# onesamblack/distributed-torch-horovod-gcp

Hardware: NVIDIA H100
Metric: images/sec (whole job, device-timed, max over ranks) ResNet-50 synthetic ImageNet training (higher is better)
Workload: dtype bf16

## Files before the change

### distributed_torch_horovod_gcp_b200/csrc/conv_sm90.cu

```cuda
#include <cuda.h>
#include <cuda_bf16.h>
#include <cuda_runtime.h>
#include <limits.h>
#include <stdint.h>
#include <stdio.h>
#include <stdlib.h>
#include <string.h>

#include "sm90_common.cuh"

namespace {

constexpr int MAX_TAPS = 9;
constexpr int MAX_CLASSES = 4;

struct ConvTap {
  int amap;
  int dw, dh;
  int wcol;
};
struct ConvClass {
  int ntaps;
  int out_map;
  ConvTap taps[MAX_TAPS];
};
struct ConvParams {
  GemmParams g;
  int num_classes;
  int kc_per_tap;
  int bw, bh, bn;
  int sw, sh;
  int tiles_w, tiles_h, tiles_n;
  int num_taps_total;
  int out_w, out_h, out_n;
  ConvClass cls[MAX_CLASSES];
};
struct alignas(64) ConvMaps {
  CUtensorMap a[4];
  CUtensorMap b;
  CUtensorMap out[4];
};

enum { MODE_FPROP = 0, MODE_DGRAD = 1, MODE_WGRAD = 2 };

template <int BN, int MODE>
struct ConvWork {
  static constexpr bool kStats = MODE == MODE_FPROP, kSplitK = MODE == MODE_WGRAD;
  static constexpr bool B_MN = MODE != MODE_FPROP;
  const ConvMaps& maps;
  const ConvParams& p;
  int nnb, pix_tiles, tiles, items, kb_per_split;

  __device__ ConvWork(const ConvMaps& maps_, const ConvParams& p_)
      : maps(maps_), p(p_), nnb(p_.g.num_n_blocks), pix_tiles(p_.tiles_w * p_.tiles_h * p_.tiles_n),
        tiles(MODE == MODE_WGRAD ? p_.g.num_m_blocks * nnb * p_.num_taps_total : p_.num_classes * pix_tiles * nnb),
        items(tiles * p_.g.splits),
        kb_per_split(MODE == MODE_WGRAD ? (pix_tiles + p_.g.splits - 1) / p_.g.splits : 0) {}
  __device__ void prefetch() const {
    for (int i = 0; i < 4; ++i) tma_prefetch_desc(&maps.a[i]);
    tma_prefetch_desc(&maps.b);
    for (int i = 0; i < 4; ++i) tma_prefetch_desc(&maps.out[i]);
  }
  __device__ int num_kb(int w) const {
    if (MODE != MODE_WGRAD) return p.cls[(w / nnb) / pix_tiles].ntaps * p.kc_per_tap;
    const int kb0 = (w / tiles) * kb_per_split;
    return min(kb0 + kb_per_split, pix_tiles) - kb0;
  }
  template <class Next>
  __device__ void load(int w, Next& next) const {
    if (MODE != MODE_WGRAD) {
      const int nt = w % nnb;
      const int rest = w / nnb;
      const int mt = rest % pix_tiles;
      const ConvClass& cl = p.cls[rest / pix_tiles];
      const int w0 = (mt % p.tiles_w) * p.bw;
      const int h0 = ((mt / p.tiles_w) % p.tiles_h) * p.bh;
      const int n0 = (mt / (p.tiles_w * p.tiles_h)) * p.bn;
      const int n_idx = nt * BN;
      for (int t = 0; t < cl.ntaps; ++t) {
        const ConvTap tap = cl.taps[t];
        for (int kc = 0; kc < p.kc_per_tap; ++kc) {
          const Stage s = next();
          tma_load_4d(&maps.a[tap.amap], s.bar, s.a, kc * BLOCK_K, w0 + tap.dw, h0 + tap.dh, n0);
          if (!B_MN) {
            tma_load_2d(&maps.b, s.bar, s.b, tap.wcol + kc * BLOCK_K, n_idx);
          } else {
#pragma unroll
            for (int c = 0; c < BN / 64; ++c)
              tma_load_2d(&maps.b, s.bar, s.b + c * (BLOCK_K * 128), tap.wcol + n_idx + 64 * c, kc * BLOCK_K);
          }
        }
      }
    } else {
      const int tile = w % tiles, split = w / tiles;
      const ConvTap tap = p.cls[0].taps[tile % p.num_taps_total];
      const int mn = tile / p.num_taps_total;
      const int m_idx = (mn / nnb) * BLOCK_M;
      const int n_idx = (mn % nnb) * BN;
      const int kb0 = split * kb_per_split;
      const int kb1 = min(kb0 + kb_per_split, pix_tiles);
      for (int kb = kb0; kb < kb1; ++kb) {
        const int w0 = (kb % p.tiles_w) * p.bw;
        const int h0 = ((kb / p.tiles_w) % p.tiles_h) * p.bh;
        const int n0 = (kb / (p.tiles_w * p.tiles_h)) * p.bn;
        const Stage s = next();
#pragma unroll
        for (int c = 0; c < BLOCK_M / 64; ++c)
          tma_load_4d(&maps.out[0], s.bar, s.a + c * (BLOCK_K * 128), m_idx + 64 * c, w0, h0, n0);
#pragma unroll
        for (int c = 0; c < BN / 64; ++c)
          tma_load_4d(&maps.a[tap.amap], s.bar, s.b + c * (BLOCK_K * 128), n_idx + 64 * c, w0 + tap.dw,
                      h0 + tap.dh, n0);
      }
    }
  }
  __device__ Slab slab(int w, int q) const {
    if (MODE != MODE_WGRAD) {
      const int nt = w % nnb;
      const int rest = w / nnb;
      const int mt = rest % pix_tiles;
      const int r0 = q * 32;
      StoreAt at;
      at.rank4 = 1;
      at.w = (mt % p.tiles_w) * p.bw + (r0 % p.bw);
      at.h = ((mt / p.tiles_w) % p.tiles_h) * p.bh + (r0 / p.bw) % p.bh;
      at.n = (mt / (p.tiles_w * p.tiles_h)) * p.bn + r0 / (p.bw * p.bh);
      at.sw = p.sw; at.sh = p.sh;
      at.vw = p.out_w - at.w; at.vh = p.out_h - at.h; at.vn = p.out_n - at.n;
      return Slab{&maps.out[p.cls[rest / pix_tiles].out_map], 0, nt * BN, at, 0, 0, 0, 0};
    }
    const int tile = w % tiles;
    const ConvTap tap = p.cls[0].taps[tile % p.num_taps_total];
    const int mn = tile / p.num_taps_total;
    const int m_idx = (mn / nnb) * BLOCK_M;
    return Slab{nullptr, m_idx + q * 32, (mn % nnb) * BN, StoreAt{}, tile, m_idx, tap.wcol, w / tiles};
  }
};

template <int BN, int MODE>
__global__ void __launch_bounds__(NUM_THREADS, 1)
conv_bf16_kernel(const __grid_constant__ ConvMaps maps, const __grid_constant__ ConvParams p) {
  persistent_body<BN, MODE == MODE_WGRAD, MODE != MODE_FPROP>(ConvWork<BN, MODE>(maps, p), p.g);
}

int make_map4(CUtensorMap* m, const void* ptr, uint64_t C, uint64_t Wd, uint64_t Hd, uint64_t Nd, uint64_t pw,
              uint64_t ph, uint64_t pn, uint32_t bw, uint32_t bh, uint32_t bn) {
  const cuuint64_t dims[4] = {C, Wd, Hd, Nd};
  const cuuint64_t strides[3] = {pw * 2, ph * 2, pn * 2};
  const cuuint32_t box[4] = {64, bw, bh, bn};
  return encode_map(m, ptr, 4, dims, strides, box);
}

void choose_box(int W, int H, int N, int rows, int* bw, int* bh, int* bn) {
  double best = 1e30;
  *bw = 1; *bh = 1; *bn = rows;
  for (int w = 1; w <= rows; w <<= 1) {
    for (int h = 1; w * h <= rows; h <<= 1) {
      const int n = rows / (w * h);
      const double covered = (double)((W + w - 1) / w * w) * ((H + h - 1) / h * h) * ((N + n - 1) / n * n);
      const double score = covered - 1e-3 * w - 1e-6 * h;
      if (score < best) { best = score; *bw = w; *bh = h; *bn = n; }
    }
  }
}

int floordiv2(int e) { return (e >= 0) ? e / 2 : -((-e + 1) / 2); }

struct ConvShape {
  int N, H, W, Cin, Cout, R, S, stride, pad, OH, OW;
};

int check_shape(ConvShape& s) {
  if (s.R != s.S || (s.R != 1 && s.R != 3)) return fail("only 1x1 and 3x3 filters");
  if (s.pad != (s.R - 1) / 2) return fail("padding must be (R-1)/2");
  if (s.stride != 1 && s.stride != 2) return fail("stride must be 1 or 2");
  if (s.stride == 2 && ((s.H | s.W) & 1)) return fail("stride 2 needs even H and W");
  if ((s.Cin % 8) || (s.Cout % 8)) return fail("channels must be multiples of 8");
  s.OH = s.H / s.stride;
  s.OW = s.W / s.stride;
  return 0;
}

int make_parity_maps(CUtensorMap* maps, const void* base, int C, int W, int H, int N, int bw, int bh, int bn) {
  for (int ph = 0; ph < 2; ++ph)
    for (int pw = 0; pw < 2; ++pw) {
      const __nv_bfloat16* ptr = reinterpret_cast<const __nv_bfloat16*>(base) + ((size_t)ph * W + pw) * C;
      if (make_map4(&maps[ph * 2 + pw], ptr, C, W / 2, H / 2, N, 2 * (uint64_t)C, 2 * (uint64_t)W * C,
                    (uint64_t)H * W * C, bw, bh, bn))
        return -1;
    }
  return 0;
}

void forward_taps(ConvClass& cl, int R, int S, int Cin, int stride, int pad) {
  for (int r = 0; r < R; ++r)
    for (int c = 0; c < S; ++c) {
      ConvTap& t = cl.taps[cl.ntaps++];
      const int eh = r - pad, ew = c - pad;
      if (stride == 1) {
        t.amap = 0; t.dh = eh; t.dw = ew;
      } else {
        const int ph = eh & 1, pw = ew & 1;
        t.amap = ph * 2 + pw; t.dh = floordiv2(eh - ph); t.dw = floordiv2(ew - pw);
      }
      t.wcol = (r * S + c) * Cin;
    }
}

void slab_box(ConvParams& p) {
  p.sw = p.bw < 32 ? p.bw : 32;
  p.sh = (32 / p.sw) < p.bh ? (32 / p.sw) : p.bh;
}

template <int MODE>
int launch_conv(const ConvMaps& maps, const ConvParams& p, int BN, int work, int max_ctas, cudaStream_t st) {
  if (BN == 64) return launch_persistent<conv_bf16_kernel<64, MODE>, 64>(work, max_ctas, st, maps, p);
  return launch_persistent<conv_bf16_kernel<128, MODE>, 128>(work, max_ctas, st, maps, p);
}

ConvParams conv_params() {
  ConvParams p;
  memset(&p, 0, sizeof(p));
  p.g.M = INT_MAX;
  p.g.splits = 1;
  p.g.alpha = 1.0f;
  return p;
}

}

extern "C" {

const char* b200dp_conv_last_error() { return g_err; }

int b200dp_conv_fprop(const void* x, const void* w, void* y, int N, int H, int W, int Cin, int Cout, int R, int S,
                      int stride, int pad, int block_n, int max_ctas, float* stats, unsigned long long stream) {
  if (ensure_init()) return -1;
  ConvShape s{N, H, W, Cin, Cout, R, S, stride, pad, 0, 0};
  if (check_shape(s)) return -1;
  if (((uintptr_t)x | (uintptr_t)w | (uintptr_t)y) & 15) return fail("pointers must be 16-byte aligned");
  const int BN = pick_bn(Cout, block_n);
  if (BN < 0) return -1;
  ConvMaps maps;
  ConvParams p = conv_params();
  p.g.N = Cout; p.g.ldc = Cout; p.g.C = y; p.g.out_mode = 0;
  p.g.stats = stats;
  if (stats != nullptr && Cout > STATS_MAX_N) return fail("stats: Cout <= 2048 required");
  p.g.num_n_blocks = (Cout + BN - 1) / BN;
  p.g.num_k_blocks = (Cin + BLOCK_K - 1) / BLOCK_K;
  p.kc_per_tap = p.g.num_k_blocks;
  choose_box(s.OW, s.OH, N, BLOCK_M, &p.bw, &p.bh, &p.bn);
  p.tiles_w = (s.OW + p.bw - 1) / p.bw; p.tiles_h = (s.OH + p.bh - 1) / p.bh; p.tiles_n = (N + p.bn - 1) / p.bn;
  p.num_classes = 1;
  p.num_taps_total = R * S;
  p.out_w = s.OW; p.out_h = s.OH; p.out_n = N;
  forward_taps(p.cls[0], R, S, Cin, stride, pad);
  if (stride == 1) {
    if (make_map4(&maps.a[0], x, Cin, W, H, N, Cin, (uint64_t)W * Cin, (uint64_t)H * W * Cin, p.bw, p.bh, p.bn))
      return -1;
    maps.a[1] = maps.a[2] = maps.a[3] = maps.a[0];
  } else if (make_parity_maps(maps.a, x, Cin, W, H, N, p.bw, p.bh, p.bn)) {
    return -1;
  }
  if (make_map2(&maps.b, w, Cout, (uint64_t)R * S * Cin, (uint64_t)R * S * Cin, BN)) return -1;
  slab_box(p);
  if (make_map4(&maps.out[0], y, Cout, s.OW, s.OH, N, Cout, (uint64_t)s.OW * Cout, (uint64_t)s.OH * s.OW * Cout, p.sw,
                p.sh, 32 / (p.sw * p.sh)))
    return -1;
  maps.out[1] = maps.out[2] = maps.out[3] = maps.out[0];
  const int work = p.tiles_w * p.tiles_h * p.tiles_n * p.g.num_n_blocks;
  return launch_conv<MODE_FPROP>(maps, p, BN, work, max_ctas, (cudaStream_t)(uintptr_t)stream);
}

int b200dp_conv_dgrad(const void* dy, const void* w, void* dx, int N, int H, int W, int Cin, int Cout, int R, int S,
                      int stride, int pad, int block_n, int max_ctas, unsigned long long stream) {
  if (ensure_init()) return -1;
  ConvShape s{N, H, W, Cin, Cout, R, S, stride, pad, 0, 0};
  if (check_shape(s)) return -1;
  if (((uintptr_t)dy | (uintptr_t)w | (uintptr_t)dx) & 15) return fail("pointers must be 16-byte aligned");
  cudaStream_t st = (cudaStream_t)(uintptr_t)stream;
  const int BN = pick_bn(Cin, block_n);
  if (BN < 0) return -1;
  ConvMaps maps;
  ConvParams p = conv_params();
  p.g.N = Cin; p.g.ldc = Cin; p.g.C = dx; p.g.out_mode = 0;
  p.g.num_n_blocks = (Cin + BN - 1) / BN;
  p.g.num_k_blocks = (Cout + BLOCK_K - 1) / BLOCK_K;
  p.kc_per_tap = p.g.num_k_blocks;
  choose_box(s.OW, s.OH, N, BLOCK_M, &p.bw, &p.bh, &p.bn);
  p.tiles_w = (s.OW + p.bw - 1) / p.bw; p.tiles_h = (s.OH + p.bh - 1) / p.bh; p.tiles_n = (N + p.bn - 1) / p.bn;
  p.num_taps_total = R * S;
  p.out_w = s.OW; p.out_h = s.OH; p.out_n = N;
  slab_box(p);
  const int sn = 32 / (p.sw * p.sh);
  if (make_map4(&maps.a[0], dy, Cout, s.OW, s.OH, N, Cout, (uint64_t)s.OW * Cout, (uint64_t)s.OH * s.OW * Cout,
                p.bw, p.bh, p.bn))
    return -1;
  maps.a[1] = maps.a[2] = maps.a[3] = maps.a[0];
// ... 91 lines not shown
```

### distributed_torch_horovod_gcp_b200/csrc/gemm_sm90.cu

```cuda
#include <cuda.h>
#include <cuda_bf16.h>
#include <cuda_runtime.h>
#include <stdint.h>

#include "sm90_common.cuh"

namespace {

template <int BN, bool A_MN, bool B_MN>
struct GemmWork {
  static constexpr bool kStats = true, kSplitK = true;
  const CUtensorMap *a, *b, *c;
  const GemmParams& p;
  int tiles, items, kb_per_split;

  __device__ GemmWork(const CUtensorMap* a_, const CUtensorMap* b_, const CUtensorMap* c_, const GemmParams& p_)
      : a(a_), b(b_), c(c_), p(p_), tiles(p_.num_m_blocks * p_.num_n_blocks), items(tiles * p_.splits),
        kb_per_split((p_.num_k_blocks + p_.splits - 1) / p_.splits) {}
  __device__ void prefetch() const {
    tma_prefetch_desc(a);
    tma_prefetch_desc(b);
    if (p.out_mode == 0) tma_prefetch_desc(c);
  }
  __device__ int m_idx(int tile) const {
    return (p.n_fastest ? tile / p.num_n_blocks : tile % p.num_m_blocks) * BLOCK_M;
  }
  __device__ int n_idx(int tile) const { return (p.n_fastest ? tile % p.num_n_blocks : tile / p.num_m_blocks) * BN; }
  __device__ int num_kb(int w) const {
    const int kb0 = (w / tiles) * kb_per_split;
    return min(kb0 + kb_per_split, p.num_k_blocks) - kb0;
  }
  template <class Next>
  __device__ void load(int w, Next& next) const {
    const int tile = w % tiles;
    const int m0 = m_idx(tile), n0 = n_idx(tile);
    const int kb0 = (w / tiles) * kb_per_split;
    const int kb1 = min(kb0 + kb_per_split, p.num_k_blocks);
    for (int kb = kb0; kb < kb1; ++kb) {
      const Stage s = next();
      const int k_idx = kb * BLOCK_K;
      if (!A_MN) {
        tma_load_2d(a, s.bar, s.a, k_idx, m0);
      } else {
#pragma unroll
        for (int c = 0; c < BLOCK_M / 64; ++c)
          tma_load_2d(a, s.bar, s.a + c * (BLOCK_K * 128), m0 + 64 * c, k_idx);
      }
      if (!B_MN) {
        tma_load_2d(b, s.bar, s.b, k_idx, n0);
      } else {
#pragma unroll
        for (int c = 0; c < BN / 64; ++c)
          tma_load_2d(b, s.bar, s.b + c * (BLOCK_K * 128), n0 + 64 * c, k_idx);
      }
    }
  }
  __device__ Slab slab(int w, int q) const {
    const int tile = w % tiles, split = w / tiles;
    const int m0 = m_idx(tile);
    return Slab{c, m0 + q * 32, n_idx(tile), StoreAt{}, tile, m0, 0, split};
  }
};

template <int BN, bool A_MN, bool B_MN>
__global__ void __launch_bounds__(NUM_THREADS, 1)
gemm_bf16_kernel(const __grid_constant__ CUtensorMap map_a, const __grid_constant__ CUtensorMap map_b,
                 const __grid_constant__ CUtensorMap map_c, const __grid_constant__ GemmParams p) {
  persistent_body<BN, A_MN, B_MN>(GemmWork<BN, A_MN, B_MN>(&map_a, &map_b, &map_c, p), p);
}

int launch_bn(int BN, int a_mn, int b_mn, const CUtensorMap& ma, const CUtensorMap& mb, const CUtensorMap& mc,
              const GemmParams& p, int max_ctas, cudaStream_t st) {
  const int work = p.num_m_blocks * p.num_n_blocks * p.splits;
#define LAUNCH(BNV, AMN, BMN) \
  launch_persistent<gemm_bf16_kernel<BNV, AMN, BMN>, BNV>(work, max_ctas, st, ma, mb, mc, p)
#define DISPATCH(BNV)                                          \
  if (BN == BNV) {                                             \
    if (!a_mn && !b_mn) return LAUNCH(BNV, false, false);      \
    if (!a_mn && b_mn) return LAUNCH(BNV, false, true);        \
    if (a_mn && !b_mn) return LAUNCH(BNV, true, false);        \
    return LAUNCH(BNV, true, true);                            \
  }
  DISPATCH(64)
  DISPATCH(128)
#undef DISPATCH
#undef LAUNCH
  return fail("unreachable");
}

}

extern "C" {

const char* b200dp_gemm_last_error() { return g_err; }

int b200dp_gemm_bf16(const void* A, const void* B, void* C, int M, int N, int K, int lda, int ldb, int ldc,
                     int a_mn, int b_mn, const void* bias_bf16, const void* bias_f32, const void* residual,
                     void* preact, int act, int out_mode, int out_bf16, float alpha, int splits, int block_n,
                     int max_ctas, float* stats, const void* res_mask, unsigned long long stream) {
  if (ensure_init()) return -1;
  if (M <= 0 || N <= 0 || K <= 0) return fail("bad shape");
  if ((N % 8) || (lda % 8) || (ldb % 8) || (ldc % 4) || ((out_mode == 0 || out_bf16) && (ldc % 8)))
    return fail("alignment: N, lda, ldb, ldc must be multiples of 8");
  if (((uintptr_t)A | (uintptr_t)B | (uintptr_t)C) & 15) return fail("pointers must be 16-byte aligned");
  const int BN = pick_bn(N, block_n);
  if (BN < 0) return -1;
  GemmParams p{};
  p.M = M; p.N = N; p.ldc = ldc;
  p.num_m_blocks = (M + BLOCK_M - 1) / BLOCK_M;
  p.num_n_blocks = (N + BN - 1) / BN;
  p.num_k_blocks = (K + BLOCK_K - 1) / BLOCK_K;
  p.splits = normalize_splits(splits, p.num_k_blocks);
  if (p.splits > 1 && (out_mode == 0 || bias_bf16 || bias_f32 || residual || preact || act))
    return fail("split-K requires out_mode 1/2 without bias, residual or activation");
  p.act = act; p.out_mode = out_mode; p.c_bf16 = out_bf16 ? 1 : 0; p.C = C; p.bias = bias_bf16; p.bias_f32 = bias_f32;
  p.residual = residual; p.preact = preact; p.alpha = alpha;
  p.stats = stats;
  p.res_mask = reinterpret_cast<const unsigned char*>(res_mask);
  if (res_mask != nullptr && (residual == nullptr || preact != nullptr || act > 2 || out_mode != 0 || (N % 64) ||
                              ldc != N))
    return fail("res_mask: plain bf16 residual, dense rows and N % 64 == 0 required");
  if (stats != nullptr && (N > STATS_MAX_N || out_mode != 0)) return fail("stats: N <= 2048 and bf16 output required");
  p.n_fastest = ((size_t)N * (size_t)K * 2 <= ((size_t)20 << 20)) ? 1 : 0;
  CUtensorMap ma, mb, mc;
  if (a_mn ? make_map2(&ma, A, K, M, lda, BLOCK_K) : make_map2(&ma, A, M, K, lda, BLOCK_M)) return -1;
  if (b_mn ? make_map2(&mb, B, K, N, ldb, BLOCK_K) : make_map2(&mb, B, N, K, ldb, BN)) return -1;
  if (out_mode == 0) {
    if (make_map2(&mc, C, M, N, ldc, 32)) return -1;
  } else {
    mc = ma;
  }
  cudaStream_t st = (cudaStream_t)(uintptr_t)stream;
  if (p.splits > 1) p.splitk_slice = (long long)M * ldc;
  return run_splitk(p, p.num_m_blocks * p.num_n_blocks, st,
                    [&] { return launch_bn(BN, a_mn, b_mn, ma, mb, mc, p, max_ctas, st); });
}

}
```

### distributed_torch_horovod_gcp_b200/csrc/sm90_common.cuh

```cuda
#pragma once
#include <cuda.h>
#include <cuda_bf16.h>
#include <cuda_runtime.h>
#include <stdint.h>
#include <stdio.h>

namespace {

constexpr int BLOCK_M = 128;
constexpr int BLOCK_K = 64;
constexpr int WGMMA_K = 16;
constexpr int NUM_THREADS = 384;
constexpr int SMEM_LIMIT = 232448;

struct GemmParams {
  int M, N;
  int ldc;
  int num_m_blocks, num_n_blocks, num_k_blocks;
  int splits;
  int act;
  int out_mode;
  int c_bf16;
  void* C;
  const void* bias;
// ... 81 lines not shown
  asm volatile("cp.async.bulk.wait_group.read %0;" ::"n"(N) : "memory");
}
__device__ __forceinline__ void tma_store_wait_all() { asm volatile("cp.async.bulk.wait_group 0;" ::: "memory"); }
__device__ __forceinline__ void fence_async_smem() { asm volatile("fence.proxy.async.shared::cta;" ::: "memory"); }
__device__ __forceinline__ void tma_prefetch_desc(const CUtensorMap* map) {
  asm volatile("prefetch.tensormap [%0];" ::"l"(map) : "memory");
}
__device__ __forceinline__ void wg_fence() { asm volatile("wgmma.fence.sync.aligned;" ::: "memory"); }
__device__ __forceinline__ void wg_commit() { asm volatile("wgmma.commit_group.sync.aligned;" ::: "memory"); }
template <int N>
__device__ __forceinline__ void wg_wait() {
  asm volatile("wgmma.wait_group.sync.aligned %0;" ::"n"(N) : "memory");
}
template <int R>
__device__ __forceinline__ void wg_fence_operands(float* d) {
#pragma unroll
  for (int i = 0; i < R; ++i) asm volatile("" : "+f"(d[i])::"memory");
}
__device__ __forceinline__ void named_bar(int id, int count) {
  asm volatile("bar.sync %0, %1;" ::"r"(id), "r"(count) : "memory");
}

template <int TA, int TB>
__device__ __forceinline__ void wgmma_bf16_n64(float* d, uint64_t a, uint64_t b, uint32_t acc) {
  asm volatile(
      "{\n\t.reg .pred p;\n\tsetp.ne.b32 p, %34, 0;\n\t"
      "wgmma.mma_async.sync.aligned.m64n64k16.f32.bf16.bf16 {%0, %1, %2, %3, %4, %5, %6, %7, %8, %9, %10, %11, %12, %13, %14, %15, %16, %17, %18, %19, %20, %21, %22, %23, %24, %25, %26, %27, %28, %29, %30, %31}, %32, %33, p, 1, 1, %35, %36;\n\t}\n"
      : "+f"(d[0]), "+f"(d[1]), "+f"(d[2]), "+f"(d[3]), "+f"(d[4]), "+f"(d[5]), "+f"(d[6]), "+f"(d[7]), "+f"(d[8]), "+f"(d[9]), "+f"(d[10]), "+f"(d[11]), "+f"(d[12]), "+f"(d[13]), "+f"(d[14]), "+f"(d[15]), "+f"(d[16]), "+f"(d[17]), "+f"(d[18]), "+f"(d[19]), "+f"(d[20]), "+f"(d[21]), "+f"(d[22]), "+f"(d[23]), "+f"(d[24]), "+f"(d[25]), "+f"(d[26]), "+f"(d[27]), "+f"(d[28]), "+f"(d[29]), "+f"(d[30]), "+f"(d[31])
      : "l"(a), "l"(b), "r"(acc), "n"(TA), "n"(TB));
}

template <int TA, int TB>
__device__ __forceinline__ void wgmma_bf16_n128(float* d, uint64_t a, uint64_t b, uint32_t acc) {
  asm volatile(
      "{\n\t.reg .pred p;\n\tsetp.ne.b32 p, %66, 0;\n\t"
      "wgmma.mma_async.sync.aligned.m64n128k16.f32.bf16.bf16 {%0, %1, %2, %3, %4, %5, %6, %7, %8, %9, %10, %11, %12, %13, %14, %15, %16, %17, %18, %19, %20, %21, %22, %23, %24, %25, %26, %27, %28, %29, %30, %31, %32, %33, %34, %35, %36, %37, %38, %39, %40, %41, %42, %43, %44, %45, %46, %47, %48, %49, %50, %51, %52, %53, %54, %55, %56, %57, %58, %59, %60, %61, %62, %63}, %64, %65, p, 1, 1, %67, %68;\n\t}\n"
      : "+f"(d[0]), "+f"(d[1]), "+f"(d[2]), "+f"(d[3]), "+f"(d[4]), "+f"(d[5]), "+f"(d[6]), "+f"(d[7]), "+f"(d[8]), "+f"(d[9]), "+f"(d[10]), "+f"(d[11]), "+f"(d[12]), "+f"(d[13]), "+f"(d[14]), "+f"(d[15]), "+f"(d[16]), "+f"(d[17]), "+f"(d[18]), "+f"(d[19]), "+f"(d[20]), "+f"(d[21]), "+f"(d[22]), "+f"(d[23]), "+f"(d[24]), "+f"(d[25]), "+f"(d[26]), "+f"(d[27]), "+f"(d[28]), "+f"(d[29]), "+f"(d[30]), "+f"(d[31]), "+f"(d[32]), "+f"(d[33]), "+f"(d[34]), "+f"(d[35]), "+f"(d[36]), "+f"(d[37]), "+f"(d[38]), "+f"(d[39]), "+f"(d[40]), "+f"(d[41]), "+f"(d[42]), "+f"(d[43]), "+f"(d[44]), "+f"(d[45]), "+f"(d[46]), "+f"(d[47]), "+f"(d[48]), "+f"(d[49]), "+f"(d[50]), "+f"(d[51]), "+f"(d[52]), "+f"(d[53]), "+f"(d[54]), "+f"(d[55]), "+f"(d[56]), "+f"(d[57]), "+f"(d[58]), "+f"(d[59]), "+f"(d[60]), "+f"(d[61]), "+f"(d[62]), "+f"(d[63])
      : "l"(a), "l"(b), "r"(acc), "n"(TA), "n"(TB));
}

__device__ __forceinline__ void wgmma_tf32_n32(float* d, uint64_t a, uint64_t b, uint32_t acc) {
  asm volatile(
      "{\n\t.reg .pred p;\n\tsetp.ne.b32 p, %18, 0;\n\t"
      "wgmma.mma_async.sync.aligned.m64n32k8.f32.tf32.tf32 {%0, %1, %2, %3, %4, %5, %6, %7, %8, %9, %10, %11, %12, %13, %14, %15}, %16, %17, p, 1, 1;\n\t}\n"
      : "+f"(d[0]), "+f"(d[1]), "+f"(d[2]), "+f"(d[3]), "+f"(d[4]), "+f"(d[5]), "+f"(d[6]), "+f"(d[7]), "+f"(d[8]), "+f"(d[9]), "+f"(d[10]), "+f"(d[11]), "+f"(d[12]), "+f"(d[13]), "+f"(d[14]), "+f"(d[15])
      : "l"(a), "l"(b), "r"(acc));
}


__device__ __forceinline__ uint64_t make_desc(uint32_t smem_addr, uint32_t lbo_bytes,
                                              uint32_t sbo_bytes) {
  uint64_t d = 0;
  d |= (uint64_t)((smem_addr & 0x3FFFF) >> 4);
  d |= (uint64_t)((lbo_bytes >> 4) & 0x3FFF) << 16;
  d |= (uint64_t)((sbo_bytes >> 4) & 0x3FFF) << 32;
  d |= (uint64_t)1 << 62;
  return d;
}

__device__ __forceinline__ bool elect_one() {
  uint32_t pred;
  asm volatile(
      "{\n\t"
      ".reg .pred p;\n\t"
      "elect.sync _|p, 0xffffffff;\n\t"
      "selp.u32 %0, 1, 0, p;\n\t"
      "}\n"
      : "=r"(pred));
  return pred != 0;
}

__device__ __forceinline__ uint64_t make_desc_base(uint32_t lbo_bytes, uint32_t sbo_bytes) {
  return make_desc(0, lbo_bytes, sbo_bytes);
}
__device__ __forceinline__ uint64_t desc_addr(uint32_t smem_addr) { return (uint64_t)((smem_addr & 0x3FFFF) >> 4); }

template <int BN, bool TA, bool TB>
__device__ __forceinline__ void wgmma_bf16(float* d, uint64_t a, uint64_t b, uint32_t acc) {
  static_assert(BN == 64 || BN == 128, "wgmma width");
  if constexpr (BN == 64) wgmma_bf16_n64<TA ? 1 : 0, TB ? 1 : 0>(d, a, b, acc);
  else wgmma_bf16_n128<TA ? 1 : 0, TB ? 1 : 0>(d, a, b, acc);
}

template <int BN, bool A_MN, bool B_MN, int STAGES, int A_BYTES, int B_BYTES>
__device__ __forceinline__ void wg_mainloop(float* d, uint32_t sa, uint32_t sb, uint64_t* full_bar, uint64_t* empty_bar,
                                            int& stage, uint32_t& phase, int nkb, int wg) {
  constexpr uint32_t KSTEP_A = A_MN ? ((WGMMA_K * 128) >> 4) : ((WGMMA_K * 2) >> 4);
  constexpr uint32_t KSTEP_B = B_MN ? ((WGMMA_K * 128) >> 4) : ((WGMMA_K * 2) >> 4);
  const uint64_t a0 = (A_MN ? make_desc_base(BLOCK_K * 128, 1024) : make_desc_base(16, 1024)) +
                      desc_addr(sa + (uint32_t)wg * 8192u);
  const uint64_t b0 = (B_MN ? make_desc_base(BLOCK_K * 128, 1024) : make_desc_base(16, 1024)) + desc_addr(sb);
  const bool leader = (threadIdx.x & 127) == 0;
  int prev = -1;
  for (int kb = 0; kb < nkb; ++kb) {
    mbar_wait(&full_bar[stage], phase);
    const uint64_t da = a0 + (uint64_t)(stage * (A_BYTES >> 4));
    const uint64_t db = b0 + (uint64_t)(stage * (B_BYTES >> 4));
    wg_fence();
#pragma unroll
    for (int k = 0; k < BLOCK_K / WGMMA_K; ++k)
      wgmma_bf16<BN, A_MN, B_MN>(d, da + k * KSTEP_A, db + k * KSTEP_B, (kb | k) ? 1u : 0u);
    wg_commit();
    wg_wait<1>();
    if (prev >= 0 && leader) mbar_arrive(&empty_bar[prev]);
    prev = stage;
    if (++stage == STAGES) { stage = 0; phase ^= 1; }
  }
  wg_wait<0>();
  wg_fence_operands<BN / 2>(d);
  if (prev >= 0 && leader) mbar_arrive(&empty_bar[prev]);
}

__device__ __forceinline__ float fast_erf(float x) {
  const float ax = fabsf(x);
  const float t = __fdividef(1.0f, fmaf(0.3275911f, ax, 1.0f));
  float poly = fmaf(1.061405429f, t, -1.453152027f);
  poly = fmaf(poly, t, 1.421413741f);
  poly = fmaf(poly, t, -0.284496736f);
  poly = fmaf(poly, t, 0.254829592f);
  const float y = 1.0f - poly * t * __expf(-ax * ax);
  return copysignf(y, x);
}
__device__ __forceinline__ float gelu_erf(float x) {
  return 0.5f * x * (1.0f + fast_erf(x * 0.70710678118654752f));
}

__device__ __forceinline__ float gelu_erf_grad(float x) {
  const float cdf = 0.5f * (1.0f + fast_erf(x * 0.70710678118654752f));
  const float pdf = 0.3989422804014327f * __expf(-0.5f * x * x);
  return cdf + x * pdf;
}

__device__ __forceinline__ void unpack8(const uint4& x, float* f) {
  const uint32_t wv[4] = {x.x, x.y, x.z, x.w};
#pragma unroll
  for (int t = 0; t < 4; ++t) {
    f[2 * t] = __uint_as_float(wv[t] << 16);
    f[2 * t + 1] = __uint_as_float(wv[t] & 0xffff0000u);
  }
}

template <int BN>
struct Cfg {
  static constexpr int A_BYTES = BLOCK_M * BLOCK_K * 2;
  static constexpr int B_BYTES = BN * BLOCK_K * 2;
  static constexpr int STAGE_BYTES = A_BYTES + B_BYTES;
  static constexpr int NCH = BN / 64;
  static constexpr int STORE_BYTES = BLOCK_M * BN * 2;
  static constexpr int FIXED_BYTES = STORE_BYTES + 1024  + 256  + STATS_SMEM_BYTES;
  static constexpr int STAGES = (SMEM_LIMIT - FIXED_BYTES) / STAGE_BYTES;
  static constexpr int SMEM_BYTES = STAGES * STAGE_BYTES + FIXED_BYTES;
  static_assert(STAGES >= 4, "shared memory");
  static_assert(2 * STAGES * 8 <= 256, "barrier space");
};

struct StoreAt {
  int rank4, w, h, n;
  int sw, sh, vw, vh, vn;
};

__device__ __forceinline__ void epi_sts128(uint32_t addr, const uint4& v) {
  asm volatile("st.shared.v4.b32 [%0], {%1, %2, %3, %4};" ::"r"(addr), "r"(v.x), "r"(v.y), "r"(v.z), "r"(v.w) : "memory");
}
__device__ __forceinline__ void epi_sts32(uint32_t addr, uint32_t v) {
  asm volatile("st.shared.b32 [%0], %1;" ::"r"(addr), "r"(v) : "memory");
}
__device__ __forceinline__ uint32_t epi_lds32(uint32_t addr) {
  uint32_t v;
  asm volatile("ld.shared.b32 %0, [%1];" : "=r"(v) : "r"(addr) : "memory");
  return v;
}
__device__ __forceinline__ uint32_t prmt_sign(uint32_t a, uint32_t sel) {
  uint32_t d;
  asm("prmt.b32 %0, %1, %2, %3;" : "=r"(d) : "r"(a), "r"(0u), "r"(sel));
  return d;
}
__device__ __forceinline__ uint32_t cvt_bf16x2(float lo, float hi) {
  uint32_t o;
  asm("cvt.rn.bf16x2.f32 %0, %1, %2;" : "=r"(o) : "f"(hi), "f"(lo));
  return o;
}
__device__ __forceinline__ float zero_plus_ftz(float v) {
  float o;
  asm("add.ftz.f32 %0, %1, %2;" : "=f"(o) : "f"(0.0f), "f"(v));
  return o;
}

template <int BN>
__device__ __forceinline__ uint32_t stage_off(int r, int u) {
  return (uint32_t)((((r >> 5) * (BN / 64) + (u >> 3)) << 12) + ((r & 31) << 7) + (((u ^ r) & 7) << 4));
}

template <int BN>
__device__ __forceinline__ void res_load(const GemmParams& p, uint4* rv, int m0, int r0, int n_idx, int lane) {
  const __nv_bfloat16* rbase = reinterpret_cast<const __nv_bfloat16*>(p.residual);
#pragma unroll
  for (int i = 0; i < BN / 16; ++i) {
    const int e = i * 32 + lane, row = m0 + r0 + e / (BN / 8), col = n_idx + (e % (BN / 8)) * 8;
    rv[i] = (row < p.M && col < p.N) ? *reinterpret_cast<const uint4*>(rbase + (size_t)row * p.ldc + col)
                                     : make_uint4(0, 0, 0, 0);
  }
  if (p.res_mask != nullptr) {
    uint32_t mbits[BN / 16];
#pragma unroll
    for (int i = 0; i < BN / 16; ++i) {
      const int e = i * 32 + lane, row = m0 + r0 + e / (BN / 8), col = n_idx + (e % (BN / 8)) * 8;
      mbits[i] = (row < p.M && col < p.N) ? (uint32_t)p.res_mask[(size_t)row * (size_t)(p.N >> 3) + (size_t)(col >> 3)]
                                          : 0u;
    }
#pragma unroll
    for (int i = 0; i < BN / 16; ++i) {
      const uint32_t rep = mbits[i] * 0x01010101u;
      const uint32_t lo = (rep & 0x08040201u) + 0x7f7f7f7fu, hi = (rep & 0x80402010u) + 0x7f7f7f7fu;
      rv[i].x &= prmt_sign(lo, 0x9988u);
      rv[i].y &= prmt_sign(lo, 0xbbaau);
      rv[i].z &= prmt_sign(hi, 0x9988u);
      rv[i].w &= prmt_sign(hi, 0xbbaau);
    }
  }
}
template <int BN>
__device__ __forceinline__ void res_stage(const uint4* rv, uint32_t stg, int r0, int lane) {
#pragma unroll
  for (int i = 0; i < BN / 16; ++i) {
    const int e = i * 32 + lane;
    epi_sts128(stg + stage_off<BN>(r0 + e / (BN / 8), e % (BN / 8)), rv[i]);
  }
}

template <int BN>
__device__ __forceinline__ void epilogue_frag(const GemmParams& p, const float* d, uint32_t stg, int wg, int m0,
                                              int n_idx, int split, long long c_off) {
  const int t = threadIdx.x & 127, lane = t & 31;
  const int r = wg * 64 + (t >> 5) * 16 + (lane >> 2);
  const uint32_t x = (uint32_t)(r & 7);
  const uint32_t sbase = stg + (uint32_t)(((r >> 5) * (BN / 64)) << 12) + (uint32_t)((r & 31) << 7) +
// ... 199 lines not shown
  }
  if (epi_tid == 0) g_stats_done = 0u;
}

__device__ __forceinline__ void splitk_finish_tile(const GemmParams& p, int tile, int m_idx, int n_idx, int bn,
                                                   long long c_off, int epi_tid, int* s_last) {
  __threadfence();
  asm volatile("bar.sync 3, 256;" ::: "memory");
  if (epi_tid == 0) *s_last = atomicAdd(p.splitk_count + tile, 1) == p.splits - 1;
  asm volatile("bar.sync 3, 256;" ::: "memory");
  if (!*s_last) return;
  __threadfence();
  const int rows = min(BLOCK_M, p.M - m_idx), c4n = min(bn, p.N - n_idx) >> 2;
  const bool add = p.out_mode == 1;
  for (int e = epi_tid; e < rows * c4n; e += 256) {
    const long long off = c_off + (long long)(m_idx + e / c4n) * p.ldc + n_idx + (e % c4n) * 4;
    float4 s = __ldcg(reinterpret_cast<const float4*>(p.splitk_ws + off));
    for (int k = 1; k < p.splits; ++k) {
      const float4 v = __ldcg(reinterpret_cast<const float4*>(p.splitk_ws + (long long)k * p.splitk_slice + off));
      s.x += v.x; s.y += v.y; s.z += v.z; s.w += v.w;
    }
    s.x = 0.0f + s.x; s.y = 0.0f + s.y; s.z = 0.0f + s.z; s.w = 0.0f + s.w;
    if (p.c_bf16) {
      uint2* c = reinterpret_cast<uint2*>(reinterpret_cast<__nv_bfloat16*>(p.C) + off);
      if (add) {
        const uint2 o = *c;
        s.x += __uint_as_float(o.x << 16); s.y += __uint_as_float(o.x & 0xffff0000u);
        s.z += __uint_as_float(o.y << 16); s.w += __uint_as_float(o.y & 0xffff0000u);
      }
      *c = make_uint2(cvt_bf16x2(s.x, s.y), cvt_bf16x2(s.z, s.w));
    } else {
      float4* c = reinterpret_cast<float4*>(reinterpret_cast<float*>(p.C) + off);
      if (add) {
        const float4 o = *c;
        s.x += o.x; s.y += o.y; s.z += o.z; s.w += o.w;
      }
      *c = s;
    }
  }
}

template <int BN>
__device__ __forceinline__ void stats_flush(const GemmParams& p, float* s_stats, int n_idx, int epi_tid) {
  constexpr int HALF = (BN >= 128) ? BN / 2 : BN;
  asm volatile("bar.sync 2, 256;" ::: "memory");
  if (epi_tid < BN) {
    const int h = epi_tid / HALF, l = epi_tid % HALF;
    const float* r = s_stats + (h * 4) * STATS_WARP_FLOATS + l;
    float s = 0.f, q = 0.f;
#pragma unroll
    for (int k = 0; k < 4; ++k) {
      s += r[k * STATS_WARP_FLOATS];
      q += r[k * STATS_WARP_FLOATS + STATS_WARP_FLOATS / 2];
    }
    if (n_idx + epi_tid < p.N) {
      float* slot = stats_slot();
      slot[n_idx + epi_tid] += s;
      slot[STATS_MAX_N + n_idx + epi_tid] += q;
    }
  }
  asm volatile("bar.sync 2, 256;" ::: "memory");
#pragma unroll
  for (int i = 0; i < 8; ++i) s_stats[i * 256 + epi_tid] = 0.f;
  asm volatile("bar.sync 2, 256;" ::: "memory");
}

struct Stage {
  uint8_t* a;
  uint8_t* b;
  uint64_t* bar;
};
struct Slab {
  const CUtensorMap* map_c;
  int m_row0, n_idx;
  StoreAt at;
  int tile;
  int m_idx;
  long long c_off;
  int split;
};

template <int BN, bool A_MN, bool B_MN, class Work>
__device__ __forceinline__ void persistent_body(const Work& wk, const GemmParams& p) {
  using C = Cfg<BN>;
  extern __shared__ __align__(1024) uint8_t smem_raw[];
  uint8_t* smem = reinterpret_cast<uint8_t*>((reinterpret_cast<uintptr_t>(smem_raw) + 1023) &
                                             ~static_cast<uintptr_t>(1023));
  uint8_t* smem_a = smem;
  uint8_t* smem_b = smem + C::STAGES * C::A_BYTES;
  uint8_t* smem_store = smem + C::STAGES * C::STAGE_BYTES;
  uint64_t* bars = reinterpret_cast<uint64_t*>(smem_store + C::STORE_BYTES);
  uint64_t* full_bar = bars;
  uint64_t* empty_bar = bars + C::STAGES;
  float* s_stats = reinterpret_cast<float*>(reinterpret_cast<uint8_t*>(bars) + 256);
  const bool want_stats = Work::kStats && p.stats != nullptr && p.out_mode == 0;
  if (want_stats) stats_zero(s_stats, NUM_THREADS, p.N);

  const int warp = threadIdx.x >> 5;
  const int lane = threadIdx.x & 31;

  if (warp == 0 && lane == 0) {
    wk.prefetch();
    for (int i = 0; i < C::STAGES; ++i) {
      mbar_init(&full_bar[i], 1);
      mbar_init(&empty_bar[i], 2);
    }
    asm volatile("fence.mbarrier_init.release.cluster;" ::: "memory");
  }
  __syncthreads();

  if (warp < 4) {
    asm volatile("setmaxnreg.dec.sync.aligned.u32 40;" ::: "memory");
    if (warp == 0 && elect_one()) {
      int stage = 0;
      uint32_t phase = 0;
      auto next = [&]() {
        mbar_wait(&empty_bar[stage], phase ^ 1);
        mbar_expect_tx(&full_bar[stage], C::STAGE_BYTES);
        const Stage s{smem_a + stage * C::A_BYTES, smem_b + stage * C::B_BYTES, &full_bar[stage]};
        if (++stage == C::STAGES) { stage = 0; phase ^= 1; }
        return s;
      };
      for (int w = blockIdx.x; w < wk.items; w += gridDim.x) wk.load(w, next);
    }
  } else {
    asm volatile("setmaxnreg.inc.sync.aligned.u32 232;" ::: "memory");
    const int cw = warp - 4;
    const int wg = cw >> 2;
    const int r0 = wg * 64 + (cw & 3) * 16;
    const int q = cw & 3;
    const int half = cw >> 2;
    const int c_begin = (BN >= 128) ? half * (BN / 2) : 0;
    const int c_end = (BN >= 128) ? c_begin + BN / 2 : (half == 0 ? BN : 0);
    const int epi_tid = cw * 32 + lane;
    float* my_stats = s_stats + cw * STATS_WARP_FLOATS;
    const uint32_t stg = smem_u32(smem_store);
    __shared__ int s_last;
    int stats_n = -1;
    int stage = 0;
    uint32_t phase = 0;
    float d[BN / 2];
    for (int w = blockIdx.x; w < wk.items; w += gridDim.x) {
      const Slab s = wk.slab(w, q);
      wg_mainloop<BN, A_MN, B_MN, C::STAGES, C::A_BYTES, C::B_BYTES>(d, smem_u32(smem_a), smem_u32(smem_b), full_bar,
                                                                     empty_bar, stage, phase, wk.num_kb(w), wg);
      if (want_stats && s.n_idx != stats_n) {
        if (stats_n >= 0) stats_flush<BN>(p, s_stats, stats_n, epi_tid);
        stats_n = s.n_idx;
      }
      const bool res = p.residual != nullptr && p.out_mode != 1;
      uint4 rv[BN / 16];
      if (res) res_load<BN>(p, rv, s.m_idx, r0, s.n_idx, lane);
      if (p.out_mode == 0) {
        if (lane == 0) tma_store_wait_read<0>();
        named_bar(1, 256);
      }
      if (res) {
        __syncwarp();
        res_stage<BN>(rv, stg, r0, lane);
        __syncwarp();
      }
      epilogue_frag<BN>(p, d, stg, wg, s.m_idx, s.n_idx, s.split, s.c_off);
      if (p.out_mode == 0) {
        fence_async_smem();
        named_bar(1, 256);
        store_slab<BN>(p, s.map_c, smem_store, q, lane, s.m_row0, s.n_idx, c_begin, c_end, s.at,
                       want_stats ? my_stats : nullptr);
      }
      if (Work::kSplitK && p.splits > 1) splitk_finish_tile(p, s.tile, s.m_idx, s.n_idx, BN, s.c_off, epi_tid, &s_last);
    }
    if (want_stats && stats_n >= 0) stats_flush<BN>(p, s_stats, stats_n, epi_tid);
    if (want_stats) stats_finalize(p, epi_tid);
    if (p.out_mode == 0 && lane == 0) tma_store_wait_all();
  }
}

typedef CUresult (*EncodeTiledFn)(CUtensorMap*, CUtensorMapDataType, cuuint32_t, void*, const cuuint64_t*,
                                  const cuuint64_t*, const cuuint32_t*, const cuuint32_t*,
                                  CUtensorMapInterleave, CUtensorMapSwizzle, CUtensorMapL2promotion,
                                  CUtensorMapFloatOOBfill);
EncodeTiledFn g_encode = nullptr;
thread_local char g_err[512];
int g_num_sms = 0;

int fail(const char* msg, int code = 0) {
  snprintf(g_err, sizeof(g_err), "%s (%d)", msg, code);
  return -1;
}

inline void bind_primary_context() {
  static thread_local bool bound = false;
  if (!bound) {
    cudaFree(nullptr);
    bound = true;
  }
}

int ensure_init() {
  bind_primary_context();
  if (g_encode) return 0;
  void* fn = nullptr;
  cudaDriverEntryPointQueryResult st;
  cudaError_t e = cudaGetDriverEntryPoint("cuTensorMapEncodeTiled", &fn, cudaEnableDefault, &st);
  if (e != cudaSuccess || st != cudaDriverEntryPointSuccess || !fn)
    return fail("cuTensorMapEncodeTiled entry point unavailable", (int)e);
  g_encode = reinterpret_cast<EncodeTiledFn>(fn);
  int dev = 0;
  cudaGetDevice(&dev);
  cudaDeviceGetAttribute(&g_num_sms, cudaDevAttrMultiProcessorCount, dev);
  return 0;
}

int encode_map(CUtensorMap* m, const void* ptr, int rank, const cuuint64_t* dims, const cuuint64_t* byte_strides,
               const cuuint32_t* box) {
  const cuuint32_t estr[4] = {1, 1, 1, 1};
  CUresult r = g_encode(m, CU_TENSOR_MAP_DATA_TYPE_BFLOAT16, rank, const_cast<void*>(ptr), dims, byte_strides, box,
                        estr, CU_TENSOR_MAP_INTERLEAVE_NONE, CU_TENSOR_MAP_SWIZZLE_128B,
                        CU_TENSOR_MAP_L2_PROMOTION_L2_256B, CU_TENSOR_MAP_FLOAT_OOB_FILL_NONE);
  if (r != CUDA_SUCCESS) return fail("cuTensorMapEncodeTiled failed", (int)r);
  return 0;
}

int make_map2(CUtensorMap* m, const void* ptr, uint64_t rows, uint64_t cols, uint64_t ld, uint32_t box_rows) {
  const cuuint64_t dims[2] = {cols, rows};
  const cuuint64_t strides[1] = {ld * 2};
  const cuuint32_t box[2] = {64, box_rows};
  return encode_map(m, ptr, 2, dims, strides, box);
}

template <auto Kernel>
int smem_attr_once(int bytes) {
  static bool attr_set = false;
  if (!attr_set) {
    cudaError_t e = cudaFuncSetAttribute(Kernel, cudaFuncAttributeMaxDynamicSharedMemorySize, bytes);
    if (e != cudaSuccess) return fail(cudaGetErrorString(e), (int)e);
    attr_set = true;
  }
  return 0;
}

template <auto Kernel, int BN, class... Args>
int launch_persistent(int work, int max_ctas, cudaStream_t st, const Args&... args) {
  if (smem_attr_once<Kernel>(Cfg<BN>::SMEM_BYTES)) return -1;
  int grid = work < g_num_sms ? work : g_num_sms;
  if (max_ctas > 0 && grid > max_ctas) grid = max_ctas;
  if (grid > STATS_MAX_CTAS) grid = STATS_MAX_CTAS;
  Kernel<<<grid, NUM_THREADS, Cfg<BN>::SMEM_BYTES, st>>>(args...);
  cudaError_t e = cudaGetLastError();
  if (e != cudaSuccess) return fail(cudaGetErrorString(e), (int)e);
  return 0;
}

template <class Launch>
int run_splitk(GemmParams& p, int tiles, cudaStream_t st, Launch&& launch) {
  void* ws = nullptr;
  if (p.splits > 1) {
    const size_t slices = (size_t)p.splits * (size_t)p.splitk_slice * sizeof(float);
    cudaError_t e = cudaMallocAsync(&ws, slices + (size_t)tiles * sizeof(int), st);
    if (e == cudaSuccess) {
      p.splitk_ws = reinterpret_cast<float*>(ws);
      p.splitk_count = reinterpret_cast<int*>(reinterpret_cast<char*>(ws) + slices);
      e = cudaMemsetAsync(p.splitk_count, 0, (size_t)tiles * sizeof(int), st);
    }
    if (e != cudaSuccess) return fail(cudaGetErrorString(e), (int)e);
  }
  const int rc = launch();
  if (ws != nullptr) {
    cudaError_t e = cudaFreeAsync(ws, st);
    if (e != cudaSuccess && rc == 0) return fail(cudaGetErrorString(e), (int)e);
  }
  return rc;
}

int normalize_splits(int splits, int kblocks) {
  if (splits > kblocks) splits = kblocks;
  if (splits < 1) splits = 1;
  const int per = (kblocks + splits - 1) / splits;
  return (kblocks + per - 1) / per;
}

int pick_bn(int n, int block_n) {
  if (block_n == 0) return n > 64 ? 128 : 64;
  if (block_n == 256) return 128;
  if (block_n != 64 && block_n != 128) return fail("block_n must be 64/128/256");
  return block_n;
}

}
```

Before: 5719.

## Keep narrow-N weight operand resident in shared memory for small-K conv/GEMM

Adds resident-B variants of the persistent conv and GEMM kernels for layers with a single 64-wide N block and at most 9 K blocks. The producer loads the whole weight operand into shared memory once per CTA behind a dedicated mbarrier. The mainloop then indexes B by k-block instead of by pipeline stage, and per-stage loads carry only the activation tile. This removes repeated weight TMA traffic and frees stage space for deeper A pipelining, at the cost of a fixed shared-memory reservation and extra template variants.

```diff
diff --git a/distributed_torch_horovod_gcp_b200/csrc/conv_sm90.cu b/distributed_torch_horovod_gcp_b200/csrc/conv_sm90.cu
--- a/distributed_torch_horovod_gcp_b200/csrc/conv_sm90.cu
+++ b/distributed_torch_horovod_gcp_b200/csrc/conv_sm90.cu
@@ -43,9 +43,10 @@
 
 enum { MODE_FPROP = 0, MODE_DGRAD = 1, MODE_WGRAD = 2 };
 
-template <int BN, int MODE>
+template <int BN, int MODE, int RESB_KB = 0>
 struct ConvWork {
   static constexpr bool kStats = MODE == MODE_FPROP, kSplitK = MODE == MODE_WGRAD;
+  static constexpr int kResB = RESB_KB;
   static constexpr bool B_MN = MODE != MODE_FPROP;
   const ConvMaps& maps;
   const ConvParams& p;
@@ -82,6 +83,7 @@
         for (int kc = 0; kc < p.kc_per_tap; ++kc) {
           const Stage s = next();
           tma_load_4d(&maps.a[tap.amap], s.bar, s.a, kc * BLOCK_K, w0 + tap.dw, h0 + tap.dh, n0);
+          if (RESB_KB > 0) continue;
           if (!B_MN) {
             tma_load_2d(&maps.b, s.bar, s.b, tap.wcol + kc * BLOCK_K, n_idx);
           } else {
@@ -114,6 +116,23 @@
       }
     }
   }
+  __device__ void load_resident_b(uint64_t* bar, uint8_t* dst) const {
+    const ConvClass& cl = p.cls[0];
+    mbar_expect_tx(bar, (uint32_t)(cl.ntaps * p.kc_per_tap * BN * BLOCK_K * 2));
+    for (int t = 0; t < cl.ntaps; ++t) {
+      const ConvTap tap = cl.taps[t];
+      for (int kc = 0; kc < p.kc_per_tap; ++kc) {
+        uint8_t* b = dst + (t * p.kc_per_tap + kc) * (BN * BLOCK_K * 2);
+        if (!B_MN) {
+          tma_load_2d(&maps.b, bar, b, tap.wcol + kc * BLOCK_K, 0);
+        } else {
+#pragma unroll
+          for (int c = 0; c < BN / 64; ++c)
+            tma_load_2d(&maps.b, bar, b + c * (BLOCK_K * 128), tap.wcol + 64 * c, kc * BLOCK_K);
+        }
+      }
+    }
+  }
   __device__ Slab slab(int w, int q) const {
     if (MODE != MODE_WGRAD) {
       const int nt = w % nnb;
@@ -143,6 +162,13 @@
   persistent_body<BN, MODE == MODE_WGRAD, MODE != MODE_FPROP>(ConvWork<BN, MODE>(maps, p), p.g);
 }
 
+constexpr int RESB_KB = 9;
+template <int MODE>
+__global__ void __launch_bounds__(NUM_THREADS, 1)
+conv_bf16_resb_kernel(const __grid_constant__ ConvMaps maps, const __grid_constant__ ConvParams p) {
+  persistent_body<64, false, MODE != MODE_FPROP>(ConvWork<64, MODE, RESB_KB>(maps, p), p.g);
+}
+
 int make_map4(CUtensorMap* m, const void* ptr, uint64_t C, uint64_t Wd, uint64_t Hd, uint64_t Nd, uint64_t pw,
               uint64_t ph, uint64_t pn, uint32_t bw, uint32_t bh, uint32_t bn) {
   const cuuint64_t dims[4] = {C, Wd, Hd, Nd};
@@ -214,6 +240,9 @@
 
 template <int MODE>
 int launch_conv(const ConvMaps& maps, const ConvParams& p, int BN, int work, int max_ctas, cudaStream_t st) {
+  if (MODE != MODE_WGRAD && BN == 64 && p.g.num_n_blocks == 1 && p.num_classes == 1 &&
+      p.cls[0].ntaps * p.kc_per_tap <= RESB_KB)
+    return launch_persistent<conv_bf16_resb_kernel<MODE>, 64, RESB_KB>(work, max_ctas, st, maps, p);
   if (BN == 64) return launch_persistent<conv_bf16_kernel<64, MODE>, 64>(work, max_ctas, st, maps, p);
   return launch_persistent<conv_bf16_kernel<128, MODE>, 128>(work, max_ctas, st, maps, p);
 }
diff --git a/distributed_torch_horovod_gcp_b200/csrc/gemm_sm90.cu b/distributed_torch_horovod_gcp_b200/csrc/gemm_sm90.cu
--- a/distributed_torch_horovod_gcp_b200/csrc/gemm_sm90.cu
+++ b/distributed_torch_horovod_gcp_b200/csrc/gemm_sm90.cu
@@ -7,9 +7,10 @@
 
 namespace {
 
-template <int BN, bool A_MN, bool B_MN>
+template <int BN, bool A_MN, bool B_MN, int RESB_KB = 0>
 struct GemmWork {
   static constexpr bool kStats = true, kSplitK = true;
+  static constexpr int kResB = RESB_KB;
   const CUtensorMap *a, *b, *c;
   const GemmParams& p;
   int tiles, items, kb_per_split;
@@ -46,12 +47,25 @@
         for (int c = 0; c < BLOCK_M / 64; ++c)
           tma_load_2d(a, s.bar, s.a + c * (BLOCK_K * 128), m0 + 64 * c, k_idx);
       }
+      if (RESB_KB > 0) continue;
       if (!B_MN) {
         tma_load_2d(b, s.bar, s.b, k_idx, n0);
       } else {
 #pragma unroll
         for (int c = 0; c < BN / 64; ++c)
           tma_load_2d(b, s.bar, s.b + c * (BLOCK_K * 128), n0 + 64 * c, k_idx);
+      }
+    }
+  }
+  __device__ void load_resident_b(uint64_t* bar, uint8_t* dst) const {
+    mbar_expect_tx(bar, (uint32_t)(p.num_k_blocks * BN * BLOCK_K * 2));
+    for (int kb = 0; kb < p.num_k_blocks; ++kb) {
+      uint8_t* d = dst + kb * (BN * BLOCK_K * 2);
+      if (!B_MN) {
+        tma_load_2d(b, bar, d, kb * BLOCK_K, 0);
+      } else {
+#pragma unroll
+        for (int c = 0; c < BN / 64; ++c) tma_load_2d(b, bar, d + c * (BLOCK_K * 128), 64 * c, kb * BLOCK_K);
       }
     }
   }
@@ -69,9 +83,21 @@
   persistent_body<BN, A_MN, B_MN>(GemmWork<BN, A_MN, B_MN>(&map_a, &map_b, &map_c, p), p);
 }
 
+constexpr int GEMM_RESB_KB = 9;
+template <bool B_MN>
+__global__ void __launch_bounds__(NUM_THREADS, 1)
+gemm_bf16_resb_kernel(const __grid_constant__ CUtensorMap map_a, const __grid_constant__ CUtensorMap map_b,
+                      const __grid_constant__ CUtensorMap map_c, const __grid_constant__ GemmParams p) {
+  persistent_body<64, false, B_MN>(GemmWork<64, false, B_MN, GEMM_RESB_KB>(&map_a, &map_b, &map_c, p), p);
+}
+
 int launch_bn(int BN, int a_mn, int b_mn, const CUtensorMap& ma, const CUtensorMap& mb, const CUtensorMap& mc,
               const GemmParams& p, int max_ctas, cudaStream_t st) {
   const int work = p.num_m_blocks * p.num_n_blocks * p.splits;
+  if (BN == 64 && !a_mn && p.num_n_blocks == 1 && p.splits == 1 && p.num_k_blocks <= GEMM_RESB_KB) {
+    if (b_mn) return launch_persistent<gemm_bf16_resb_kernel<true>, 64, GEMM_RESB_KB>(work, max_ctas, st, ma, mb, mc, p);
+    return launch_persistent<gemm_bf16_resb_kernel<false>, 64, GEMM_RESB_KB>(work, max_ctas, st, ma, mb, mc, p);
+  }
 #define LAUNCH(BNV, AMN, BMN) \
   launch_persistent<gemm_bf16_kernel<BNV, AMN, BMN>, BNV>(work, max_ctas, st, ma, mb, mc, p)
 #define DISPATCH(BNV)                                          \
diff --git a/distributed_torch_horovod_gcp_b200/csrc/sm90_common.cuh b/distributed_torch_horovod_gcp_b200/csrc/sm90_common.cuh
--- a/distributed_torch_horovod_gcp_b200/csrc/sm90_common.cuh
+++ b/distributed_torch_horovod_gcp_b200/csrc/sm90_common.cuh
@@ -187,7 +187,7 @@
   else wgmma_bf16_n128<TA ? 1 : 0, TB ? 1 : 0>(d, a, b, acc);
 }
 
-template <int BN, bool A_MN, bool B_MN, int STAGES, int A_BYTES, int B_BYTES>
+template <int BN, bool A_MN, bool B_MN, int STAGES, int A_BYTES, int B_BYTES, bool RES_B = false>
 __device__ __forceinline__ void wg_mainloop(float* d, uint32_t sa, uint32_t sb, uint64_t* full_bar, uint64_t* empty_bar,
                                             int& stage, uint32_t& phase, int nkb, int wg) {
   constexpr uint32_t KSTEP_A = A_MN ? ((WGMMA_K * 128) >> 4) : ((WGMMA_K * 2) >> 4);
@@ -200,7 +200,7 @@
   for (int kb = 0; kb < nkb; ++kb) {
     mbar_wait(&full_bar[stage], phase);
     const uint64_t da = a0 + (uint64_t)(stage * (A_BYTES >> 4));
-    const uint64_t db = b0 + (uint64_t)(stage * (B_BYTES >> 4));
+    const uint64_t db = b0 + (uint64_t)((RES_B ? kb : stage) * (B_BYTES >> 4));
     wg_fence();
 #pragma unroll
     for (int k = 0; k < BLOCK_K / WGMMA_K; ++k)
@@ -245,18 +245,19 @@
   }
 }
 
-template <int BN>
+template <int BN, int RESB_KB = 0>
 struct Cfg {
   static constexpr int A_BYTES = BLOCK_M * BLOCK_K * 2;
   static constexpr int B_BYTES = BN * BLOCK_K * 2;
-  static constexpr int STAGE_BYTES = A_BYTES + B_BYTES;
+  static constexpr int RES_B_BYTES = RESB_KB * B_BYTES;
+  static constexpr int STAGE_BYTES = A_BYTES + (RESB_KB ? 0 : B_BYTES);
   static constexpr int NCH = BN / 64;
   static constexpr int STORE_BYTES = BLOCK_M * BN * 2;
-  static constexpr int FIXED_BYTES = STORE_BYTES + 1024  + 256  + STATS_SMEM_BYTES;
+  static constexpr int FIXED_BYTES = STORE_BYTES + 1024  + 256  + STATS_SMEM_BYTES + RES_B_BYTES;
   static constexpr int STAGES = (SMEM_LIMIT - FIXED_BYTES) / STAGE_BYTES;
   static constexpr int SMEM_BYTES = STAGES * STAGE_BYTES + FIXED_BYTES;
   static_assert(STAGES >= 4, "shared memory");
-  static_assert(2 * STAGES * 8 <= 256, "barrier space");
+  static_assert(2 * STAGES * 8 + 8 <= 256, "barrier space");
 };
 
 struct StoreAt {
@@ -622,13 +623,14 @@
 
 template <int BN, bool A_MN, bool B_MN, class Work>
 __device__ __forceinline__ void persistent_body(const Work& wk, const GemmParams& p) {
-  using C = Cfg<BN>;
+  using C = Cfg<BN, Work::kResB>;
+  constexpr bool RES_B = Work::kResB > 0;
   extern __shared__ __align__(1024) uint8_t smem_raw[];
   uint8_t* smem = reinterpret_cast<uint8_t*>((reinterpret_cast<uintptr_t>(smem_raw) + 1023) &
                                              ~static_cast<uintptr_t>(1023));
   uint8_t* smem_a = smem;
   uint8_t* smem_b = smem + C::STAGES * C::A_BYTES;
-  uint8_t* smem_store = smem + C::STAGES * C::STAGE_BYTES;
+  uint8_t* smem_store = smem_b + (RES_B ? C::RES_B_BYTES : C::STAGES * C::B_BYTES);
   uint64_t* bars = reinterpret_cast<uint64_t*>(smem_store + C::STORE_BYTES);
   uint64_t* full_bar = bars;
   uint64_t* empty_bar = bars + C::STAGES;
@@ -645,6 +647,7 @@
       mbar_init(&full_bar[i], 1);
       mbar_init(&empty_bar[i], 2);
     }
+    if (RES_B) mbar_init(&bars[2 * C::STAGES], 1);
     asm volatile("fence.mbarrier_init.release.cluster;" ::: "memory");
   }
   __syncthreads();
@@ -661,6 +664,7 @@
         if (++stage == C::STAGES) { stage = 0; phase ^= 1; }
         return s;
       };
+      if constexpr (RES_B) wk.load_resident_b(&bars[2 * C::STAGES], smem_b);
       for (int w = blockIdx.x; w < wk.items; w += gridDim.x) wk.load(w, next);
     }
   } else {
@@ -680,9 +684,10 @@
     int stage = 0;
     uint32_t phase = 0;
     float d[BN / 2];
+    if constexpr (RES_B) mbar_wait(&bars[2 * C::STAGES], 0);
     for (int w = blockIdx.x; w < wk.items; w += gridDim.x) {
       const Slab s = wk.slab(w, q);
-      wg_mainloop<BN, A_MN, B_MN, C::STAGES, C::A_BYTES, C::B_BYTES>(d, smem_u32(smem_a), smem_u32(smem_b), full_bar,
+      wg_mainloop<BN, A_MN, B_MN, C::STAGES, C::A_BYTES, C::B_BYTES, RES_B>(d, smem_u32(smem_a), smem_u32(smem_b), full_bar,
                                                                      empty_bar, stage, phase, wk.num_kb(w), wg);
       if (want_stats && s.n_idx != stats_n) {
         if (stats_n >= 0) stats_flush<BN>(p, s_stats, stats_n, epi_tid);
@@ -779,13 +784,13 @@
   return 0;
 }
 
-template <auto Kernel, int BN, class... Args>
+template <auto Kernel, int BN, int RESB_KB = 0, class... Args>
 int launch_persistent(int work, int max_ctas, cudaStream_t st, const Args&... args) {
-  if (smem_attr_once<Kernel>(Cfg<BN>::SMEM_BYTES)) return -1;
+  if (smem_attr_once<Kernel>(Cfg<BN, RESB_KB>::SMEM_BYTES)) return -1;
   int grid = work < g_num_sms ? work : g_num_sms;
   if (max_ctas > 0 && grid > max_ctas) grid = max_ctas;
   if (grid > STATS_MAX_CTAS) grid = STATS_MAX_CTAS;
-  Kernel<<<grid, NUM_THREADS, Cfg<BN>::SMEM_BYTES, st>>>(args...);
+  Kernel<<<grid, NUM_THREADS, Cfg<BN, RESB_KB>::SMEM_BYTES, st>>>(args...);
   cudaError_t e = cudaGetLastError();
   if (e != cudaSuccess) return fail(cudaGetErrorString(e), (int)e);
   return 0;
```

Result: no change. 5744 (median of 6 runs) (+0.4%).
